# zhaozijie2022/LocoTouch

Measured on AMD Instinct MI355X. Metric: env-steps/sec (whole node), TransportTeacher 4096 envs/GPU, higher is better.
Workload: dtype f32

## Files before the change

locotouch_amd/_abi.py:

```python
from __future__ import annotations

import ctypes
import os
import re

_HERE = os.path.dirname(os.path.abspath(__file__))
REPO = os.path.dirname(_HERE)
LIB_PATH = os.environ.get("LOCOTOUCH_AMD_LIB", os.path.join(_HERE, "_lib", "liblocotouch_env.so"))

_SCALARS = {"int": ctypes.c_int, "int32_t": ctypes.c_int32, "int64_t": ctypes.c_int64, "uint8_t": ctypes.c_uint8,
            "uint32_t": ctypes.c_uint32, "uint64_t": ctypes.c_uint64, "size_t": ctypes.c_size_t, "float": ctypes.c_float,
            "double": ctypes.c_double}
_DECL = re.compile(r"(?:const\s+)?(\w+)\s*((?:\*\s*(?:const\b\s*)?)*)(\w*)\s*((?:\[[^\]]*\]\s*)*)")


def _ctype(decl, structs, opaque, consts, typed, param):
    m = _DECL.fullmatch(decl.strip())
    if not m:
        return None
    base, stars, name, dims = m.groups()
    depth = stars.count("*")
    try:
        dims = [sum(int(t) if t.strip().isdigit() else consts[t.strip()] for t in d.split("+")) for d in re.findall(r"\[([^\]]*)\]", dims)]
    except KeyError:
# ... 91 lines not shown
    ("MEMORY_GRU", "lt_memory_gru.h", False, ("lt_memory_gru_seq_backward_units",),
     ("lt_memory_gru_net", "lt_memory_gru_seq_net", "lt_memory_gru_seq_grad")),
    ("POLICY", "lt_policy.h", True, ("lt_policy_step_launches",), ("lt_policy_desc", "lt_policy_memory")),
    ("PPO_OPTS", "lt_ppo_opts.h", False, (), ()),
    ("MLP_DX", "lt_mlp_dx.h", True, (), ()),
    ("PPO_SYM", "lt_ppo_sym.h", False, (), ()),
    ("PPO_MIRROR", "lt_ppo_mirror.h", False, (), ()),
    ("MLP_ROWS", "lt_mlp_rows.h", True, (), ()),
    ("ENCODER", "lt_encoder.h", False, ("lt_encoder_forward_launches",), ("lt_encoder_desc", "lt_encoder_net")),
    ("RNN_ENCODER", "lt_rnn_encoder.h", False, ("lt_rnn_encoder_forward_launches",),
     ("lt_rnn_encoder_memory", "lt_rnn_encoder_net")),
    ("RNN_ENCODER_TRAIN", "lt_rnn_encoder_train.h", "lt_rnn_encoder.h", ("lt_rnn_encoder_backward_launches",),
     ("lt_rnn_encoder_grad",)),
    ("POLICY_ENCODER", "lt_policy_encoder.h", False, ("lt_policy_encoder_step_launches",),
     ("lt_policy_encoder_desc", "lt_policy_encoder_params")),
)


def _bind(table, include_dir):
    bound, seen, env_structs, structs_of = [], set(), None, {}
    for prefix, fname, uses_env_structs, queries, _ in table:
        path, queries = os.path.join(include_dir, fname), frozenset(queries)
        given = structs_of[uses_env_structs] if isinstance(uses_env_structs, str) else env_structs if uses_env_structs else None
        consts, structs, sigs = parse_header(open(path).read(), structs=given, bases={"lt_cfg": _CfgMethods})
        structs_of[fname] = structs
        if not prefix:
            env_structs = structs
        for name in sorted(queries - set(sigs)):
            raise ImportError(f"include/{fname}: the value query {name} named in _abi.HEADERS is not declared there")
        for name, (restype, _) in sigs.items():
# ... 117 lines not shown
```

locotouch_amd/csrc/lt_ppo.hip:

```cpp
#include <hip/hip_runtime.h>
#include <math.h>
#include <stdint.h>

#include "lt_env.h"
#include "lt_host_check.h"
#include "lt_internal.h"
#include "lt_ppo_device.h"

namespace {

template <bool LOG, bool NORM>
__global__ __launch_bounds__(256) void lt_ppo_loss_kernel(const float* __restrict__ mu, const float* __restrict__ stdp, const float* __restrict__ value,
                                                          const float* __restrict__ actions, const float* __restrict__ old_logp,
                                                          const float* __restrict__ adv, const float* __restrict__ returns,
                                                          const float* __restrict__ old_values, const float* __restrict__ old_mu,
                                                          const float* __restrict__ old_sigma, const long long* __restrict__ idx,
                                                          long long M, int A, float clip, float vcoef, int clipped_value,
                                                          const float* __restrict__ adv_stats, float* __restrict__ dmu, float* __restrict__ dvalue, float* __restrict__ acc) {
  const long long row = (long long)blockIdx.x * 256 + threadIdx.x;
  const bool ok = row < M;
  const long long src = (ok && idx) ? idx[row] : row;
  __shared__ float sigma_lds[MAX_A];
  if constexpr (LOG) {
    if ((int)threadIdx.x < A) sigma_lds[threadIdx.x] = lt_sigma_of_log(stdp[threadIdx.x]);
// ... 157 lines not shown
      else if (J.out1[j]) J.out1[j][ei - split] = o[i];
    }
  }
}

void launch_one_sum(const float* ws, int nblk, long long stride, int count, int split, float* out0, float* out1, hipStream_t stream) {
  SumJobs J = {};
  J.njobs = 1;
  J.ws[0] = ws; J.out0[0] = out0; J.out1[0] = out1; J.stride[0] = stride;
  J.nblk[0] = nblk; J.count[0] = count; J.split[0] = split;
  const int epb = 256 / sum_row_lanes(nblk) * 4;
  J.first[1] = (count + epb - 1) / epb;
  hipLaunchKernelGGL(lt_partial_sums_kernel, dim3((unsigned)J.first[1]), dim3(256), 0, stream, J);
}

constexpr int HW_ROWS = 96, HW_MAX_N = 16;

template <int NN>
__global__ __launch_bounds__(256) void lt_head_wgrad_kernel(const float* __restrict__ dy, const float* __restrict__ x, int x_split, long long M, int n, int k,
                                                            float* __restrict__ ws) {
  const int k4 = k >> 2, lanes = 256 / k4;
  const int c4 = threadIdx.x % k4, rl = threadIdx.x / k4;
  const long long r0 = (long long)blockIdx.x * HW_ROWS;
  float4 acc[NN];
  float accb[NN];
#pragma unroll
  for (int j = 0; j < NN; ++j) { acc[j] = {0.f, 0.f, 0.f, 0.f}; accb[j] = 0.f; }
  if (rl < lanes) {
    for (int r = rl; r < HW_ROWS; r += 4 * lanes) {
      float4 xv[4];
      float d[4][NN];
#pragma unroll
      for (int u = 0; u < 4; ++u) {
        const long long row = r0 + r + u * lanes;
        const bool ok = (r + u * lanes) < HW_ROWS && row < M;
        xv[u] = ok ? ((const float4*)(x + row * k))[c4] : float4{0.f, 0.f, 0.f, 0.f};
        if (x_split) {
          const unsigned w[4] = {__float_as_uint(xv[u].x), __float_as_uint(xv[u].y), __float_as_uint(xv[u].z), __float_as_uint(xv[u].w)};
          float f[4];
#pragma unroll
          for (int i = 0; i < 4; ++i)
            f[i] = (float)__builtin_bit_cast(_Float16, (unsigned short)(w[i] & 0xFFFFu)) + (float)__builtin_bit_cast(_Float16, (unsigned short)(w[i] >> 16)) * (1.f / 64.f);
          xv[u] = float4{f[0], f[1], f[2], f[3]};
        }
#pragma unroll
        for (int j = 0; j < NN; ++j) d[u][j] = (ok && j < n) ? dy[row * n + j] : 0.f;
      }
#pragma unroll
      for (int u = 0; u < 4; ++u)
#pragma unroll
        for (int j = 0; j < NN; ++j) {
          acc[j].x += d[u][j] * xv[u].x; acc[j].y += d[u][j] * xv[u].y; acc[j].z += d[u][j] * xv[u].z; acc[j].w += d[u][j] * xv[u].w;
          accb[j] += d[u][j];
        }
    }
  }
  extern __shared__ float4 red[];
  float* const redb = (float*)(red + (size_t)lanes * NN * k4);
  if (rl < lanes) {
#pragma unroll
    for (int j = 0; j < NN; ++j) red[((size_t)rl * NN + j) * k4 + c4] = acc[j];
    if (c4 == 0)
#pragma unroll
      for (int j = 0; j < NN; ++j) redb[rl * NN + j] = accb[j];
  }
  __syncthreads();
  float* const out = ws + (size_t)blockIdx.x * ((size_t)n * k + HW_MAX_N);
  for (int e = threadIdx.x; e < n * k4; e += 256) {
    const int j = e / k4, c = e - j * k4;
    float4 t = red[(size_t)j * k4 + c];
    for (int l = 1; l < lanes; ++l) {
      const float4 u = red[((size_t)l * NN + j) * k4 + c];
      t.x += u.x; t.y += u.y; t.z += u.z; t.w += u.w;
    }
    ((float4*)(out + (size_t)j * k))[c] = t;
  }
  if (threadIdx.x < n) {
    float t = redb[threadIdx.x];
    for (int l = 1; l < lanes; ++l) t += redb[l * NN + threadIdx.x];
    out[(size_t)n * k + threadIdx.x] = t;
  }
}

__global__ __launch_bounds__(256) void lt_gae_kernel(const float* __restrict__ rewards, const unsigned char* __restrict__ dones,
                                                     const float* __restrict__ values, const float* __restrict__ last_values, float gamma,
                                                     float lam, int T, long long N, float* __restrict__ returns, float* __restrict__ advantages) {
  const long long e = (long long)blockIdx.x * 256 + threadIdx.x;
  if (e >= N) return;
  float next_v = last_values[e], gae = 0.f;
  for (int t = T - 1; t >= 0; --t) {
    const long long o = (long long)t * N + e;
    const float v = values[o], alive = 1.f - (float)dones[o];
    const float delta = rewards[o] + alive * gamma * next_v - v;
    gae = delta + alive * gamma * lam * gae;
    const float ret = gae + v;
    returns[o] = ret;
// ... 122 lines not shown
}
static int elu_backward_bias(const float* da, const float* a, int64_t M, int N, float alpha, float* dz, float* db, float* ws, float* amax, void* stream) {
  if (!da || !a || !dz || !ws || M < 1 || N < 4 || (N & 3) || N > 1024)
    return einval("lt_elu_backward_bias: invalid argument (N a multiple of 4, 4 <= N <= 1024)");
  const int nblk = (int)((M + EB_ROWS - 1) / EB_ROWS);
  hipLaunchKernelGGL(lt_elu_bwd_bias_kernel, dim3((unsigned)nblk), dim3(256), 0, (hipStream_t)stream, da, a, (long long)M, N, alpha, dz, ws, amax);
  if (db) launch_one_sum(ws, nblk, (long long)N, N, N, db, nullptr, (hipStream_t)stream);
  return launch_status();
}

extern "C" int64_t lt_head_wgrad_ws_floats(int64_t M, int n, int k) { return ((M + HW_ROWS - 1) / HW_ROWS) * ((int64_t)n * k + HW_MAX_N); }

extern "C" int lt_head_wgrad(const float* dy, const float* x, int x_split, int64_t M, int n, int k, float* dw, float* db, float* ws, void* stream) {
  if (!dy || !x || !ws || M < 1 || n < 1 || n > HW_MAX_N || k < 4 || (k & 3) || k > 1024)
    return einval("lt_head_wgrad: invalid argument (1 <= n <= 16, k a multiple of 4, 4 <= k <= 1024)");
  const int nblk = (int)((M + HW_ROWS - 1) / HW_ROWS), k4 = k / 4, lanes = 256 / k4;
  const int nn = n <= 1 ? 1 : (n <= 4 ? 4 : (n <= 8 ? 8 : (n <= 12 ? 12 : 16)));
  const size_t lds = (size_t)lanes * nn * k4 * 16 + (size_t)lanes * nn * 4;
  if (const int e = lt_ensure_dynamic_lds((const void*)lt_head_wgrad_kernel<16>, 72 * 1024)) {
    lt_set_error(hipGetErrorString((hipError_t)e));
    return LT_EHIP;
  }
  if (lds > 72 * 1024) return einval("lt_head_wgrad: n * k too large for one block's LDS partials");
  const dim3 g((unsigned)nblk), b(256);
  hipStream_t st = (hipStream_t)stream;
  switch (nn) {
    case 1: hipLaunchKernelGGL(lt_head_wgrad_kernel<1>, g, b, lds, st, dy, x, x_split, (long long)M, n, k, ws); break;
    case 4: hipLaunchKernelGGL(lt_head_wgrad_kernel<4>, g, b, lds, st, dy, x, x_split, (long long)M, n, k, ws); break;
    case 8: hipLaunchKernelGGL(lt_head_wgrad_kernel<8>, g, b, lds, st, dy, x, x_split, (long long)M, n, k, ws); break;
    case 12: hipLaunchKernelGGL(lt_head_wgrad_kernel<12>, g, b, lds, st, dy, x, x_split, (long long)M, n, k, ws); break;
    default: hipLaunchKernelGGL(lt_head_wgrad_kernel<16>, g, b, lds, st, dy, x, x_split, (long long)M, n, k, ws); break;
  }
  if (dw) launch_one_sum(ws, nblk, (long long)n * k + HW_MAX_N, n * k + n, n * k, dw, db, st);
// ... 134 lines not shown
```

locotouch_amd/rl/flat_adam.py:

```python
from __future__ import annotations

import torch

from .. import _abi


class FlatAdam:
    ALIGN = 64

    def __init__(self, optimizer: torch.optim.Adam):
        if type(optimizer) is not torch.optim.Adam or len(optimizer.param_groups) != 1:
            raise TypeError("FlatAdam wraps a single-group torch.optim.Adam")
        g = optimizer.param_groups[0]
        if g.get("amsgrad") or g.get("maximize") or g.get("capturable") or g.get("differentiable"):
            raise TypeError("FlatAdam: amsgrad / maximize / capturable / differentiable are not supported")
        self.optimizer = optimizer
        self.params = [p for p in g["params"] if p.requires_grad]
        if not self.params or any(p.dtype != torch.float32 or not p.is_cuda for p in self.params):
            raise TypeError("FlatAdam needs f32 CUDA parameters")
        self.offsets, off = [], 0
        for p in self.params:
            self.offsets.append(off)
            off += -(-p.numel() // self.ALIGN) * self.ALIGN
        self.n = off
# ... 56 lines not shown
        return self.flat_g

    def grad_views(self) -> dict:
        if not self._bound():
            self._adopt()
        for p, v in zip(self.params, self._gviews):
            p.grad = v
        return {p: v for p, v in zip(self.params, self._gviews)}

    def offset_of(self, param) -> int:
        for p, off in zip(self.params, self.offsets):
            if p is param:
                return off
        raise KeyError("parameter not in the flat bucket")

    def step_dev(self, max_norm: float, lr_dev: torch.Tensor) -> None:
        if not self._bound():
            self._adopt()
        g = self.optimizer.param_groups[0]
        self.step_count += 1
        b1, b2 = g["betas"]
        _abi.call("lt_adam_clip_step_dev", self.flat_p, self.flat_g, self.flat_m, self.flat_v, self.n, float(max_norm or 0.0), lr_dev,
                  float(b1), float(b2), float(g["eps"]), float(g["weight_decay"]), self.step_count, self._ws, self.grad_norm,
                  _abi.stream(self.flat_p.device))
        self._step_t.fill_(float(self.step_count))

    def step(self, max_norm: float, gathered: bool = False) -> None:
        if not self._bound():
            self._adopt()
        if not gathered:
            self.gather_grads()
        g = self.optimizer.param_groups[0]
        self.step_count += 1
        b1, b2 = g["betas"]
        _abi.call("lt_adam_clip_step", self.flat_p, self.flat_g, self.flat_m, self.flat_v, self.n, float(max_norm or 0.0), float(g["lr"]),
                  float(b1), float(b2), float(g["eps"]), float(g["weight_decay"]), self.step_count, self._ws, self.grad_norm,
                  _abi.stream(self.flat_p.device))
        self._step_t.fill_(float(self.step_count))
```

locotouch_amd/rl/mlp.py:

```python
from __future__ import annotations

import ctypes
import os

import torch
import torch.nn as nn

from .. import _abi

USE_FUSED_BACKWARD = os.environ.get("LT_FUSED_BACKWARD", "1") != "0"
USE_DX_KERNEL = os.environ.get("LT_MLP_DX_KERNEL", "1") != "0"
_ACT_IDS = {nn.ELU: "LT_ACT_ELU", nn.ReLU: "LT_ACT_RELU", nn.Tanh: "LT_ACT_TANH", nn.Identity: "LT_ACT_NONE"}


def describe(seq: nn.Sequential):
    linears, acts = [], set()
    mods = list(seq)
    for i, m in enumerate(mods):
        if isinstance(m, nn.Linear):
            if m.bias is None or m.weight.dtype != torch.float32:
                return None
            linears.append(m)
        elif type(m) in _ACT_IDS:
            if type(m) is nn.ELU and (m.alpha != 1.0):
# ... 231 lines not shown
            torch.mm(dz.detach(), w.detach(), out=dx_out)


class PackedPair:

    def __init__(self, actor: nn.Sequential, critic: nn.Sequential):
        self.a, self.b = PackedMLP(actor), PackedMLP(critic)
        self.check_domain = False
        self.domain_max: torch.Tensor | None = None
        self.acts_split = False
        self._bpacked_fresh = False
        self._dx_fresh = False
        self.last_backward: str | None = None
        self._bwd_shapes_ok: bool | None = None
        self.sat: torch.Tensor | None = None
        for net in (self.a, self.b):
            dims = [net.desc.dims[i] for i in range(net.desc.num_layers + 1)]
            if any(d % 4 for d in dims[1:-1]) or net.desc.activation != _abi.CONSTS["LT_ACT_ELU"]:
                raise ValueError("PackedPair: ELU stacks with hidden widths that are multiples of 4")

    def arm_domain_check(self) -> None:
        self.check_domain = True

    def _record_domain(self, tensors) -> None:
        self.check_domain = False
        with torch.no_grad():
            m_ = torch.stack([t.abs().max().float() for t in tensors]).max()
            self.domain_max = m_ if self.domain_max is None else torch.maximum(self.domain_max, m_)

    def domain_violated(self) -> bool:
# ... 74 lines not shown
            x_split_rows, xsp = (self.split_rows(x0), self.split_rows(x1)), 1
        if xsp:
            xs = x_split_rows
        dys = [d if d.is_contiguous() else d.contiguous() for d in (dy0, dy1)]
        dev = x0.device
        if self.sat is None:
            self.sat = torch.zeros(1, device=dev, dtype=torch.float32)
        if ms[0] == ms[1]:
            nblks = (lib.lt_mlp_backward_blocks(ctypes.byref(nets[0].desc), ctypes.byref(nets[1].desc), ms[0]),) * 2
        else:
            if dx_out is not None:
                raise ValueError("PackedPair: input gradients (dx_out) are served for inputs of equal row counts only")
            blocks = (ctypes.c_int64(), ctypes.c_int64())
            _abi.call("lt_mlp_backward_blocks_rows", nets[0].desc, nets[1].desc, ms[0], ms[1], ctypes.byref(blocks[0]), ctypes.byref(blocks[1]))
            nblks = (blocks[0].value, blocks[1].value)
        dzs, amaxs, arrs = [], [], []
        per_net = (SumJobs(), SumJobs()) if after_first is not None else (sums, sums)
        for k, net in enumerate(nets):
            if not self._bpacked_fresh:
                net.pack_backward()
            L = len(net.linears)
            m, nblk = ms[k], nblks[k]
            n, kk = dys[k].shape[1], acts[k][L - 2].shape[1]
            ws = torch.empty(lib.lt_head_wgrad_ws_floats(m, n, kk), device=dev, dtype=torch.float32)
            _abi.call("lt_head_wgrad", dys[k], acts[k][L - 2], asp, m, n, kk, None, None, ws, stream)
            per_net[k].add(ws, lib.lt_head_wgrad_nblk(m), n * kk + 16, n * kk + n, n * kk, grad_of[net.linears[L - 1].weight], grad_of[net.linears[L - 1].bias])
            dz = [torch.empty_like(a) for a in acts[k]]
            am = torch.empty(L - 1, nblk, device=dev, dtype=torch.float32)
            dzs.append(dz)
            amaxs.append(am)
            arrs.append((_abi.ptr_array(acts[k]), _abi.ptr_array(dz), _abi.ptr_array([am[l] for l in range(L - 1)])))
        dzsp = int(dy_amax is not None)
        scales = torch.empty(2, device=dev, dtype=torch.float32)
        in_amax = dy_amax if dzsp else (None, None)
        dx_kernel = dx_out is not None and self._dx_kernel_ok()
        if dx_kernel and not self._dx_fresh:
            self.pack_training(with_backward=True, with_dx=True)
        chain = (nets[0].desc, nets[0].bpacked, dys[0], *arrs[0], nets[1].desc, nets[1].bpacked, dys[1], *arrs[1],
                 *(ms[:1] if ms[0] == ms[1] else ms), asp, in_amax[0], in_amax[1], dzsp, scales, self.sat)
        if ms[0] != ms[1]:
            _abi.call("lt_mlp_backward_pair_rows", *chain, stream)
        elif dx_kernel:
            _abi.call("lt_mlp_backward_pair_dx", *chain, dx_out[0], dx_out[1], stream)
        else:
            _abi.call("lt_mlp_backward_pair", *chain, stream)
            if dx_out is not None:
# ... 56 lines not shown
```

locotouch_amd/rl/ppo.py:

```python
from __future__ import annotations

import torch
import torch.nn as nn

from .. import _abi
from .dist import Dist
from .modules import ActorCritic
from .storage import RolloutStorage


class PPO:
    def __init__(self, actor_critic: ActorCritic, num_learning_epochs=1, num_mini_batches=1, clip_param=0.2, gamma=0.998,
                 lam=0.95, value_loss_coef=1.0, entropy_coef=0.0, learning_rate=1e-3, max_grad_norm=1.0,
                 use_clipped_value_loss=True, schedule="fixed", desired_kl=0.01, device="cpu",
                 normalize_advantage_per_mini_batch=False, dist: Dist | None = None, rnd_cfg: dict | None = None,
                 symmetry_cfg: dict | None = None, **unused):
        if rnd_cfg is not None:
            raise NotImplementedError("rnd_cfg: random network distillation is not built (DESIGN.md §7: it needs an `rnd_state` observation "
                                      "group no env here produces); pass rnd_cfg=None")
        self.symmetry = self._resolve_symmetry(symmetry_cfg, actor_critic)
        self._sym_tables = None
        self.device = device
        self.dist = dist or Dist()
        self.actor_critic = actor_critic.to(device)
        on_gpu = torch.device(device).type == "cuda"
        self.fused_loss = on_gpu and bool(unused.get("fused_loss", True))
        self.packed_forward = on_gpu and bool(unused.get("packed_forward", True))
        self.direct_update = on_gpu and bool(unused.get("direct_update", True))
        self.fused_recurrent_update = bool(unused.get("fused_recurrent_update", False))
        self.fused_gru_memories = bool(unused.get("fused_gru_memories", False))
        self.direct_recurrent_update = bool(unused.get("direct_recurrent_update", False))
        self.fused_encoder_policy = bool(unused.get("fused_encoder_policy", False))
        self._encoders = None
        self.direct_rnn_encoder_update = bool(unused.get("direct_rnn_encoder_update", False))
        self._rnn_encoders = None
        if type(actor_critic).__name__ == "ActorCriticRNNEncoder":
            for key in ("fused_encoder_policy", "direct_recurrent_update", "fused_recurrent_update"):
                if getattr(self, key):
                    raise ValueError(f"{key}: the policy is an ActorCriticRNNEncoder: its update is the eager one (the key serves "
                                     f"{'ActorCriticEncoder' if key == 'fused_encoder_policy' else 'ActorCriticRecurrent'})")
        if self.fused_encoder_policy:
            if self.fused_recurrent_update or self.direct_recurrent_update or self.fused_gru_memories:
                raise ValueError("fused_encoder_policy: the recurrent keys (fused_recurrent_update, direct_recurrent_update, fused_gru_memories) "
# ... 198 lines not shown
            if self._adaptive:
                self._apply_kl(self.dist.all_reduce_mean_end(kl_handle), reduced=True)
            self._optim_step()
            stats = stats + torch.stack((value_loss, surrogate_loss, ent.detach()))
        n = self.num_learning_epochs * self.num_mini_batches
        sv, ss, se = (stats / n).tolist()
        if pair is not None and pair.domain_violated():
            self._warn_mlp_domain()
        st.clear()
        return sv, ss, se, None, None

    def _direct_update(self, pair, split_buckets: bool = True):
        ac, fa, sym = self.actor_critic, self._flat_adam, self.symmetry
        perm, m = self.storage.mini_batch_permutation(self.num_mini_batches)
        c = self._direct_begin("direct_update", pair, perm, m, symmetric=sym is not None)
        obs, cobs, dev, grad_of = c.obs, c.cobs, c.dev, c.grad_of
        critic_at = fa.offset_of(next(iter(ac.critic.parameters())))
        two_buckets = split_buckets and 0 < critic_at < self._flat_grad.numel()
        sym_args = None
        mirror_only = sym is not None and not sym["use_data_augmentation"]
        if sym is None:
            rows = crows = m
            perm_o, perm_co = obs[perm], cobs[perm]
            if perm_o.dtype != torch.float32:
                perm_o, perm_co = perm_o.float(), perm_co.float()
        elif mirror_only:
            rows, crows = 2 * m, m
            tab_o, _, tab_a = self._symmetry_tables(dev, obs.shape[1], None, c.a_dim)
            perm_o, perm_co = self._symmetry_gather(obs, perm, m, tab_o), cobs[perm]
            if perm_co.dtype != torch.float32:
# ... 14 lines not shown
            (mu, value), acts = pair.forward_raw(o, co)
            dmu, dvalue, acc = self._direct_loss_and_rule(c, mu, value, idx, m, i, sym_args)
            if brows != rows:
                o, dmu, acts = o[:brows], dmu[:brows], ([a[:brows] for a in acts[0]], acts[1])
            if self.dist.world_size > 1 and two_buckets:
                handles = []
                pair.backward_raw(o, co, acts, dmu, dvalue, grad_of, xs, after_first=lambda: handles.append(self.dist.all_reduce_mean_begin(self._flat_grad[:critic_at])),
                                  dy_amax=(acc[20:21], acc[21:22]))
                handles.append(self.dist.all_reduce_mean_begin(self._flat_grad[critic_at:] if handles else self._flat_grad))
                for h in handles:
                    self.dist.all_reduce_mean_end(h)
            else:
                pair.backward_raw(o, co, acts, dmu, dvalue, grad_of, xs, dy_amax=(acc[20:21], acc[21:22]))
                if self.dist.world_size > 1:
                    self.dist.all_reduce_mean_(self._flat_grad)
            fa.step_dev(self.max_grad_norm, c.lr_dev)
        return self._direct_end(c, with_dx=False)

    def _direct_begin(self, key: str, pair, index, m: int, symmetric: bool = False):
        from types import SimpleNamespace

        from .fused_loss import adv_stats, std_param

        obs, cobs, small = self._flat_storage()
        small = [t.view(-1) if t.shape[-1] == 1 else t for t in small]
        a_dim = small[0].shape[1]
        if a_dim > 16:
            raise ValueError(f"{key}: the action width is {a_dim}: the loss kernel serves at most 16")
        dev = obs.device
        state = torch.zeros(5 if symmetric else 4, device=dev)
        state[0] = self.learning_rate
        std_p, std_is_log = std_param(self.actor_critic)
        pair.arm_domain_check()
        mb_stats = adv_stats(small[2], index, m, self.num_mini_batches) if self.normalize_advantage_per_mini_batch else None
        return SimpleNamespace(pair=pair, obs=obs, cobs=cobs, small=small, a_dim=a_dim, dev=dev, state=state, lr_dev=state[:1], stats=state[1:4],
                               grad_of=self._flat_adam.grad_views(), std_p=std_p, std_is_log=std_is_log, std_c=std_p.detach(),
                               stream=_abi.stream(dev), mb_stats=mb_stats)

    def _direct_loss_and_rule(self, c, mu, value, idx, m: int, i: int, sym_args=None):
        dev = c.dev
        dmu = torch.empty_like(mu)
        dvalue = torch.empty(value.shape[0], 1, device=dev, dtype=torch.float32)
        acc = torch.empty(24, device=dev, dtype=torch.float32)
        out = torch.empty(24, device=dev, dtype=torch.float32)
        rows = (mu, c.std_c, value, *c.small, idx, m, c.a_dim, float(self.clip_param), float(self.value_loss_coef), float(self.entropy_coef),
                int(bool(self.use_clipped_value_loss)))
        opts = (int(c.std_is_log), None if c.mb_stats is None else c.mb_stats[i])
        if sym_args is not None:
            _abi.call(sym_args[0], *rows, *opts, *sym_args[1:], dmu, dvalue, acc, out, c.state[4:5], c.stream)
        elif c.std_is_log or c.mb_stats is not None:
            _abi.call("lt_ppo_loss_opts", *rows, *opts, dmu, dvalue, acc, out, c.stream)
        else:
            _abi.call("lt_ppo_loss", *rows, dmu, dvalue, acc, out, c.stream)
        kl = None
        if self._adaptive:
            kl = out[4:5]
            if self.dist.world_size > 1:
                kl = self.dist.all_reduce_mean_(kl.clone())
        _abi.call("lt_ppo_lr_rule", kl, float(self.desired_kl or 0.0), 1e-5, 1e-2, 1.5, c.lr_dev, c.stats, out, c.grad_of[c.std_p], c.a_dim, c.stream)
        return dmu, dvalue, acc

    def _direct_end(self, c, with_dx: bool):
        pair, state = c.pair, c.state
        sat, dom = pair.saturated(), pair.domain_max
        pair.domain_max = None
        zero = state.new_zeros(1)
        read = torch.cat((state, zero if sat is None else sat, zero if dom is None else dom.view(1))).tolist()
        (lr, sv, ss, se), (nsat, dmax) = read[:4], read[-2:]
        if nsat > 0:
            import warnings

            sat.zero_()
            entry = "lt_mlp_backward_pair_dx" if with_dx and pair._dx_kernel_ok() else "lt_mlp_backward_pair"
            warnings.warn(f"{entry}: {int(nsat)} workgroup-layers of the gradient chain reached the f16 image's bound "
                          "(a gradient grew by more than 500x through the layers): those rows were saturated; set LT_FUSED_BACKWARD=0 "
                          "to run the chain as f32 library GEMMs")
        self.learning_rate = lr
        for group in self.optimizer.param_groups:
# ... 545 lines not shown
```

Baseline: 68.62 million.

## Fuse PPO loss, partial sums and LR rule into one step; pair head wgrad launches

Adds a new loss-step entry point. It computes the PPO loss rows, staging per-row tensors through LDS tiles, and writes per-block partials. A tail kernel then reduces those partials and applies the adaptive LR rule and std gradient, replacing the separate loss, sum and lr_rule launches. The two networks' head weight-gradient kernels are merged into one paired launch, and the Adam step-count publish moves to once per update instead of every mini-batch. The aim is to cut kernel launches and host overhead per mini-batch, at the cost of new code paths that only apply to the non-symmetric, non-log-std, no-per-minibatch-norm case.

```diff
diff --git a/include/lt_ppo_step.h b/include/lt_ppo_step.h
--- /dev/null
+++ b/include/lt_ppo_step.h
@@ -0,0 +1,26 @@
+#ifndef LT_PPO_STEP_H
+#define LT_PPO_STEP_H
+
+#include <stddef.h>
+#include <stdint.h>
+
+#ifdef __cplusplus
+extern "C" {
+#endif
+
+int lt_ppo_loss_step_ws_floats(int64_t M);
+
+int lt_ppo_loss_step(const float* mu, const float* std, const float* value, const float* actions, const float* old_logp, const float* adv,
+                     const float* returns, const float* old_values, const float* old_mu, const float* old_sigma, const int64_t* idx, int64_t M,
+                     int A, float clip, float value_loss_coef, float entropy_coef, int use_clipped_value_loss, int std_is_log,
+                     const float* adv_stats, float desired_kl, float lr_min, float lr_max, float factor, float* lr, float* stats,
+                     float* dstd_out, float* dmu, float* dvalue, float* partials, float* acc, float* out, void* stream);
+
+int lt_head_wgrad_pair(const float* dy0, const float* x0, int64_t M0, int n0, int k0, float* ws0, const float* dy1, const float* x1, int64_t M1,
+                       int n1, int k1, float* ws1, int x_split, void* stream);
+
+#ifdef __cplusplus
+}
+#endif
+
+#endif
diff --git a/locotouch_amd/_abi.py b/locotouch_amd/_abi.py
--- a/locotouch_amd/_abi.py
+++ b/locotouch_amd/_abi.py
@@ -129,6 +129,7 @@
      ("lt_rnn_encoder_grad",)),
     ("POLICY_ENCODER", "lt_policy_encoder.h", False, ("lt_policy_encoder_step_launches",),
      ("lt_policy_encoder_desc", "lt_policy_encoder_params")),
+    ("PPO_STEP", "lt_ppo_step.h", False, ("lt_ppo_loss_step_ws_floats",), ()),
 )
 
 
diff --git a/locotouch_amd/csrc/lt_head_wgrad_device.h b/locotouch_amd/csrc/lt_head_wgrad_device.h
--- /dev/null
+++ b/locotouch_amd/csrc/lt_head_wgrad_device.h
@@ -0,0 +1,80 @@
+#pragma once
+
+#include <hip/hip_runtime.h>
+
+namespace {
+
+constexpr int HW_ROWS = 96, HW_MAX_N = 16;
+
+template <int NN>
+__device__ __forceinline__ void lt_head_wgrad_block(const float* __restrict__ dy, const float* __restrict__ x, int x_split, long long M, int n, int k,
+                                                    float* __restrict__ ws, long long blk, float4* red) {
+  const int k4 = k >> 2, lanes = 256 / k4;
+  const int c4 = threadIdx.x % k4, rl = threadIdx.x / k4;
+  const long long r0 = blk * HW_ROWS;
+  float4 acc[NN];
+  float accb[NN];
+#pragma unroll
+  for (int j = 0; j < NN; ++j) { acc[j] = {0.f, 0.f, 0.f, 0.f}; accb[j] = 0.f; }
+  if (rl < lanes) {
+    for (int r = rl; r < HW_ROWS; r += 4 * lanes) {
+      float4 xv[4];
+      float d[4][NN];
+#pragma unroll
+      for (int u = 0; u < 4; ++u) {
+        const long long row = r0 + r + u * lanes;
+        const bool ok = (r + u * lanes) < HW_ROWS && row < M;
+        xv[u] = ok ? ((const float4*)(x + row * k))[c4] : float4{0.f, 0.f, 0.f, 0.f};
+        if (x_split) {
+          const unsigned w[4] = {__float_as_uint(xv[u].x), __float_as_uint(xv[u].y), __float_as_uint(xv[u].z), __float_as_uint(xv[u].w)};
+          float f[4];
+#pragma unroll
+          for (int i = 0; i < 4; ++i)
+            f[i] = (float)__builtin_bit_cast(_Float16, (unsigned short)(w[i] & 0xFFFFu)) + (float)__builtin_bit_cast(_Float16, (unsigned short)(w[i] >> 16)) * (1.f / 64.f);
+          xv[u] = float4{f[0], f[1], f[2], f[3]};
+        }
+#pragma unroll
+        for (int j = 0; j < NN; ++j) d[u][j] = (ok && j < n) ? dy[row * n + j] : 0.f;
+      }
+#pragma unroll
+      for (int u = 0; u < 4; ++u)
+#pragma unroll
+        for (int j = 0; j < NN; ++j) {
+          acc[j].x += d[u][j] * xv[u].x; acc[j].y += d[u][j] * xv[u].y; acc[j].z += d[u][j] * xv[u].z; acc[j].w += d[u][j] * xv[u].w;
+          accb[j] += d[u][j];
+        }
+    }
+  }
+  float* const redb = (float*)(red + (size_t)lanes * NN * k4);
+  if (rl < lanes) {
+#pragma unroll
+    for (int j = 0; j < NN; ++j) red[((size_t)rl * NN + j) * k4 + c4] = acc[j];
+    if (c4 == 0)
+#pragma unroll
+      for (int j = 0; j < NN; ++j) redb[rl * NN + j] = accb[j];
+  }
+  __syncthreads();
+  float* const out = ws + (size_t)blk * ((size_t)n * k + HW_MAX_N);
+  for (int e = threadIdx.x; e < n * k4; e += 256) {
+    const int j = e / k4, c = e - j * k4;
+    float4 t = red[(size_t)j * k4 + c];
+    for (int l = 1; l < lanes; ++l) {
+      const float4 u = red[((size_t)l * NN + j) * k4 + c];
+      t.x += u.x; t.y += u.y; t.z += u.z; t.w += u.w;
+    }
+    ((float4*)(out + (size_t)j * k))[c] = t;
+  }
+  if (threadIdx.x < n) {
+    float t = redb[threadIdx.x];
+    for (int l = 1; l < lanes; ++l) t += redb[l * NN + threadIdx.x];
+    out[(size_t)n * k + threadIdx.x] = t;
+  }
+}
+
+__host__ __device__ inline int lt_head_wgrad_nn(int n) { return n <= 1 ? 1 : (n <= 4 ? 4 : (n <= 8 ? 8 : (n <= 12 ? 12 : 16))); }
+inline size_t lt_head_wgrad_lds(int n, int k) {
+  const int k4 = k / 4, lanes = 256 / k4, nn = lt_head_wgrad_nn(n);
+  return (size_t)lanes * nn * k4 * 16 + (size_t)lanes * nn * 4;
+}
+
+}
diff --git a/locotouch_amd/csrc/lt_ppo.hip b/locotouch_amd/csrc/lt_ppo.hip
--- a/locotouch_amd/csrc/lt_ppo.hip
+++ b/locotouch_amd/csrc/lt_ppo.hip
@@ -3,6 +3,7 @@
 #include <stdint.h>
 
 #include "lt_env.h"
+#include "lt_head_wgrad_device.h"
 #include "lt_host_check.h"
 #include "lt_internal.h"
 #include "lt_ppo_device.h"
@@ -195,72 +196,11 @@
   hipLaunchKernelGGL(lt_partial_sums_kernel, dim3((unsigned)J.first[1]), dim3(256), 0, stream, J);
 }
 
-constexpr int HW_ROWS = 96, HW_MAX_N = 16;
-
 template <int NN>
 __global__ __launch_bounds__(256) void lt_head_wgrad_kernel(const float* __restrict__ dy, const float* __restrict__ x, int x_split, long long M, int n, int k,
                                                             float* __restrict__ ws) {
-  const int k4 = k >> 2, lanes = 256 / k4;
-  const int c4 = threadIdx.x % k4, rl = threadIdx.x / k4;
-  const long long r0 = (long long)blockIdx.x * HW_ROWS;
-  float4 acc[NN];
-  float accb[NN];
-#pragma unroll
-  for (int j = 0; j < NN; ++j) { acc[j] = {0.f, 0.f, 0.f, 0.f}; accb[j] = 0.f; }
-  if (rl < lanes) {
-    for (int r = rl; r < HW_ROWS; r += 4 * lanes) {
-      float4 xv[4];
-      float d[4][NN];
-#pragma unroll
-      for (int u = 0; u < 4; ++u) {
-        const long long row = r0 + r + u * lanes;
-        const bool ok = (r + u * lanes) < HW_ROWS && row < M;
-        xv[u] = ok ? ((const float4*)(x + row * k))[c4] : float4{0.f, 0.f, 0.f, 0.f};
-        if (x_split) {
-          const unsigned w[4] = {__float_as_uint(xv[u].x), __float_as_uint(xv[u].y), __float_as_uint(xv[u].z), __float_as_uint(xv[u].w)};
-          float f[4];
-#pragma unroll
-          for (int i = 0; i < 4; ++i)
-            f[i] = (float)__builtin_bit_cast(_Float16, (unsigned short)(w[i] & 0xFFFFu)) + (float)__builtin_bit_cast(_Float16, (unsigned short)(w[i] >> 16)) * (1.f / 64.f);
-          xv[u] = float4{f[0], f[1], f[2], f[3]};
-        }
-#pragma unroll
-        for (int j = 0; j < NN; ++j) d[u][j] = (ok && j < n) ? dy[row * n + j] : 0.f;
-      }
-#pragma unroll
-      for (int u = 0; u < 4; ++u)
-#pragma unroll
-        for (int j = 0; j < NN; ++j) {
-          acc[j].x += d[u][j] * xv[u].x; acc[j].y += d[u][j] * xv[u].y; acc[j].z += d[u][j] * xv[u].z; acc[j].w += d[u][j] * xv[u].w;
-          accb[j] += d[u][j];
-        }
-    }
-  }
   extern __shared__ float4 red[];
-  float* const redb = (float*)(red + (size_t)lanes * NN * k4);
-  if (rl < lanes) {
-#pragma unroll
-    for (int j = 0; j < NN; ++j) red[((size_t)rl * NN + j) * k4 + c4] = acc[j];
-    if (c4 == 0)
-#pragma unroll
-      for (int j = 0; j < NN; ++j) redb[rl * NN + j] = accb[j];
-  }
-  __syncthreads();
-  float* const out = ws + (size_t)blockIdx.x * ((size_t)n * k + HW_MAX_N);
-  for (int e = threadIdx.x; e < n * k4; e += 256) {
-    const int j = e / k4, c = e - j * k4;
-    float4 t = red[(size_t)j * k4 + c];
-    for (int l = 1; l < lanes; ++l) {
-      const float4 u = red[((size_t)l * NN + j) * k4 + c];
-      t.x += u.x; t.y += u.y; t.z += u.z; t.w += u.w;
-    }
-    ((float4*)(out + (size_t)j * k))[c] = t;
-  }
-  if (threadIdx.x < n) {
-    float t = redb[threadIdx.x];
-    for (int l = 1; l < lanes; ++l) t += redb[l * NN + threadIdx.x];
-    out[(size_t)n * k + threadIdx.x] = t;
-  }
+  lt_head_wgrad_block<NN>(dy, x, x_split, M, n, k, ws, (long long)blockIdx.x, red);
 }
 
 __global__ __launch_bounds__(256) void lt_gae_kernel(const float* __restrict__ rewards, const unsigned char* __restrict__ dones,
@@ -413,9 +353,8 @@
 extern "C" int lt_head_wgrad(const float* dy, const float* x, int x_split, int64_t M, int n, int k, float* dw, float* db, float* ws, void* stream) {
   if (!dy || !x || !ws || M < 1 || n < 1 || n > HW_MAX_N || k < 4 || (k & 3) || k > 1024)
     return einval("lt_head_wgrad: invalid argument (1 <= n <= 16, k a multiple of 4, 4 <= k <= 1024)");
-  const int nblk = (int)((M + HW_ROWS - 1) / HW_ROWS), k4 = k / 4, lanes = 256 / k4;
-  const int nn = n <= 1 ? 1 : (n <= 4 ? 4 : (n <= 8 ? 8 : (n <= 12 ? 12 : 16)));
-  const size_t lds = (size_t)lanes * nn * k4 * 16 + (size_t)lanes * nn * 4;
+  const int nblk = (int)((M + HW_ROWS - 1) / HW_ROWS), nn = lt_head_wgrad_nn(n);
+  const size_t lds = lt_head_wgrad_lds(n, k);
   if (const int e = lt_ensure_dynamic_lds((const void*)lt_head_wgrad_kernel<16>, 72 * 1024)) {
     lt_set_error(hipGetErrorString((hipError_t)e));
     return LT_EHIP;
diff --git a/locotouch_amd/csrc/lt_ppo_step.hip b/locotouch_amd/csrc/lt_ppo_step.hip
--- /dev/null
+++ b/locotouch_amd/csrc/lt_ppo_step.hip
@@ -0,0 +1,311 @@
+#include <hip/hip_runtime.h>
+#include <math.h>
+#include <stdint.h>
+
+#include "lt_env.h"
+#include "lt_head_wgrad_device.h"
+#include "lt_host_check.h"
+#include "lt_internal.h"
+#include "lt_ppo_device.h"
+#include "lt_ppo_step.h"
+
+namespace {
+
+constexpr int LS_ROWS = 256;
+constexpr int LS_SLOTS = 24;
+constexpr int LS_WAVES = LS_ROWS / 64;
+constexpr int LS_TAIL_CHUNK = 128;
+
+__host__ __device__ inline int ls_stride(int A, int vec) { return vec ? (((A >> 2) & 1) ? A : A + 4) : (A | 1); }
+
+template <bool TO_LDS, typename G>
+__device__ __forceinline__ void ls_move_rows(float* __restrict__ tile, G g, int nrows, int A, int S, int vec) {
+  if (vec) {
+    const int a4 = A >> 2, nq = nrows * a4;
+    for (int q = threadIdx.x; q < nq; q += LS_ROWS) {
+      const int r = q / a4, p = q - r * a4;
+      float4* const l = (float4*)(tile + r * S + 4 * p);
+      if constexpr (TO_LDS) *l = *(const float4*)(g(r) + 4 * p);
+      else *(float4*)(g(r) + 4 * p) = *l;
+    }
+  } else {
+    const int ne = nrows * A;
+    for (int e = threadIdx.x; e < ne; e += LS_ROWS) {
+      const int r = e / A, a = e - r * A;
+      if constexpr (TO_LDS) tile[r * S + a] = g(r)[a];
+      else g(r)[a] = tile[r * S + a];
+    }
+  }
+}
+
+__device__ __forceinline__ void ls_own_row(const float* __restrict__ tile, int A, int S, int vec, float (&o)[MAX_A]) {
+  const float* const p = tile + (int)threadIdx.x * S;
+  if (vec) {
+#pragma unroll
+    for (int c = 0; c < MAX_A / 4; ++c) {
+      if (4 * c < A) {
+        const float4 v = *(const float4*)(p + 4 * c);
+        o[4 * c] = v.x; o[4 * c + 1] = v.y; o[4 * c + 2] = v.z; o[4 * c + 3] = v.w;
+      }
+    }
+  } else {
+#pragma unroll
+    for (int a = 0; a < MAX_A; ++a)
+      if (a < A) o[a] = p[a];
+  }
+}
+
+__device__ __forceinline__ float ls_inv_sigma(float sg) {
+#pragma clang fp reciprocal(off)
+  return 1.f / sg;
+}
+
+template <bool LOG, bool NORM>
+__global__ __launch_bounds__(LS_ROWS) void lt_ppo_loss_rows_kernel(const float* __restrict__ mu, const float* __restrict__ stdp, const float* __restrict__ value,
+                                                                   const float* __restrict__ actions, const float* __restrict__ old_logp,
+                                                                   const float* __restrict__ adv, const float* __restrict__ returns,
+                                                                   const float* __restrict__ old_values, const float* __restrict__ old_mu,
+                                                                   const float* __restrict__ old_sigma, const long long* __restrict__ idx,
+                                                                   long long M, int A, float clip, float vcoef, int clipped_value,
+                                                                   const float* __restrict__ adv_stats, int vec, float* __restrict__ dmu,
+                                                                   float* __restrict__ dvalue, float* __restrict__ partials) {
+  extern __shared__ float4 tiles4[];
+  __shared__ long long s_src[LS_ROWS];
+  __shared__ float sigma_lds[MAX_A];
+  __shared__ float red[LS_WAVES][4 + MAX_A];
+  __shared__ float redm[LS_WAVES][2];
+  const int S = ls_stride(A, vec);
+  float* const t_mu = (float*)tiles4;
+  float* const t_act = t_mu + LS_ROWS * S;
+  float* const t_omu = t_act + LS_ROWS * S;
+  float* const t_osg = t_omu + LS_ROWS * S;
+  const long long r0 = (long long)blockIdx.x * LS_ROWS, row = r0 + threadIdx.x;
+  const int nrows = (int)(M - r0 < LS_ROWS ? M - r0 : LS_ROWS);
+  const bool ok = (int)threadIdx.x < nrows;
+  const long long src = (ok && idx) ? idx[row] : row;
+  s_src[threadIdx.x] = src;
+  if constexpr (LOG) {
+    if ((int)threadIdx.x < A) sigma_lds[threadIdx.x] = lt_sigma_of_log(stdp[threadIdx.x]);
+  }
+  float v = 0.f, R = 0.f, olp = 0.f, advr = 0.f, ov_own = 0.f;
+  if (ok) { v = value[row]; R = returns[src]; olp = old_logp[src]; advr = adv[src]; ov_own = old_values[src]; }
+  const float* const mu_blk = mu + r0 * A;
+  ls_move_rows<true>(t_mu, [&](int r) { return mu_blk + (long long)r * A; }, nrows, A, S, vec);
+  __syncthreads();
+  ls_move_rows<true>(t_act, [&](int r) { return actions + s_src[r] * A; }, nrows, A, S, vec);
+  ls_move_rows<true>(t_omu, [&](int r) { return old_mu + s_src[r] * A; }, nrows, A, S, vec);
+  ls_move_rows<true>(t_osg, [&](int r) { return old_sigma + s_src[r] * A; }, nrows, A, S, vec);
+  __syncthreads();
+  float part[4 + MAX_A];
+  float amax_mu = 0.f, amax_v = 0.f;
+#pragma unroll
+  for (int i = 0; i < 4 + MAX_A; ++i) part[i] = 0.f;
+  if (ok) {
+    const float inv_m = 1.f / (float)M;
+    float logp = 0.f, kl = 0.f;
+    float z[MAX_A], isg[MAX_A], rm[MAX_A], rx[MAX_A], rom[MAX_A], ros[MAX_A];
+    ls_own_row(t_mu, A, S, vec, rm);
+    ls_own_row(t_act, A, S, vec, rx);
+    ls_own_row(t_omu, A, S, vec, rom);
+    ls_own_row(t_osg, A, S, vec, ros);
+#pragma unroll
+    for (int a = 0; a < MAX_A; ++a) {
+      if (a < A) {
+        const float sg = LOG ? sigma_lds[a] : stdp[a], m = rm[a], x = rx[a];
+        const float om = rom[a], os = ros[a];
+        isg[a] = ls_inv_sigma(sg);
+        z[a] = (x - m) * isg[a];
+        logp += lt_ppo_logp_term<LOG>(z[a], sg, stdp[a]);
+        kl += lt_ppo_kl_term(sg, os, om, m);
+      }
+    }
+    if constexpr (NORM) advr = (advr - adv_stats[0]) * adv_stats[1];
+    const float ratio = __expf(logp - olp);
+    LT_PPO_SURROGATE(advr, ratio, clip, s1, s2, dsurr_dratio)
+    const float dlogp = dsurr_dratio * ratio * inv_m;
+    float* const my_dmu = t_mu + (int)threadIdx.x * S;
+#pragma unroll
+    for (int a = 0; a < MAX_A; ++a) {
+      if (a < A) {
+        my_dmu[a] = dlogp * z[a] * isg[a];
+        amax_mu = fmaxf(amax_mu, fabsf(dlogp * z[a] * isg[a]));
+        if constexpr (LOG) part[4 + a] = dlogp * (z[a] * z[a] - 1.f);
+        else part[4 + a] = dlogp * (z[a] * z[a] - 1.f) * isg[a];
+      }
+    }
+    float vl, dv;
+    LT_PPO_VALUE_LOSS(v, R, &ov_own, 0, clip, clipped_value, vl, dv)
+    dvalue[row] = vcoef * dv * inv_m;
+    amax_v = fabsf(vcoef * dv * inv_m);
+    part[0] = fmaxf(s1, s2);
+    part[1] = vl;
+    part[2] = kl;
+  }
+  const int lane = threadIdx.x & 63, wave = threadIdx.x >> 6;
+#pragma unroll
+  for (int i = 0; i < 4 + MAX_A; ++i) {
+    float s = part[i];
+#pragma unroll
+    for (int off = 32; off > 0; off >>= 1) s += __shfl_xor(s, off, 64);
+    if (lane == 0) red[wave][i] = s;
+  }
+#pragma unroll
+  for (int off = 32; off > 0; off >>= 1) {
+    amax_mu = fmaxf(amax_mu, __shfl_xor(amax_mu, off, 64));
+    amax_v = fmaxf(amax_v, __shfl_xor(amax_v, off, 64));
+  }
+  if (lane == 0) { redm[wave][0] = amax_mu; redm[wave][1] = amax_v; }
+  __syncthreads();
+  float* const dmu_blk = dmu + r0 * A;
+  ls_move_rows<false>(t_mu, [&](int r) { return dmu_blk + (long long)r * A; }, nrows, A, S, vec);
+  if (threadIdx.x < LS_SLOTS) {
+    const int i = threadIdx.x;
+    float s = 0.f;
+    if (i < 4 + A && i != 3) {
+      s = red[0][i];
+#pragma unroll
+      for (int w = 1; w < LS_WAVES; ++w) s += red[w][i];
+    } else if (i == 20 || i == 21) {
+#pragma unroll
+      for (int w = 0; w < LS_WAVES; ++w) s = fmaxf(s, redm[w][i - 20]);
+    }
+    partials[(long long)blockIdx.x * LS_SLOTS + i] = s;
+  }
+}
+
+__global__ __launch_bounds__(256) void lt_ppo_loss_tail_kernel(const float* __restrict__ partials, int nblk, const float* __restrict__ stdp, int A, float inv_m,
+                                                               float vcoef, float ecoef, int std_is_log, float desired, float lr_min, float lr_max,
+                                                               float factor, float* __restrict__ lr, float* __restrict__ stats,
+                                                               float* __restrict__ dstd_out, float* __restrict__ acc, float* __restrict__ out) {
+  __shared__ float s_part[LS_TAIL_CHUNK * LS_SLOTS];
+  __shared__ float s_acc[LS_SLOTS], s_out[LS_SLOTS];
+  const int t = threadIdx.x;
+  const bool is_max = t == 20 || t == 21;
+  float s = 0.f;
+  for (int b0 = 0; b0 < nblk; b0 += LS_TAIL_CHUNK) {
+    const int nb = nblk - b0 < LS_TAIL_CHUNK ? nblk - b0 : LS_TAIL_CHUNK;
+    for (int e = t; e < nb * LS_SLOTS; e += 256) s_part[e] = partials[(long long)b0 * LS_SLOTS + e];
+    __syncthreads();
+    if (t < LS_SLOTS) {
+      if (is_max) for (int b = 0; b < nb; ++b) s = fmaxf(s, s_part[b * LS_SLOTS + t]);
+      else for (int b = 0; b < nb; ++b) s += s_part[b * LS_SLOTS + t];
+    }
+    __syncthreads();
+  }
+  if (t < LS_SLOTS) { s_acc[t] = s; acc[t] = s; s_out[t] = 0.f; }
+  __syncthreads();
+  if (t < 64) lt_ppo_finalize(s_acc, stdp, A, inv_m, vcoef, ecoef, std_is_log, s_out);
+  __syncthreads();
+  if (out && (t < 5 || (t >= 8 && t < 8 + A))) out[t] = s_out[t];
+  if (dstd_out && t < A) dstd_out[t] = s_out[8 + t];
+  if (t != 0) return;
+  if (lr && desired > 0.f) {
+#pragma clang fp reciprocal(off)
+    const float kl = s_out[4];
+    float v = *lr;
+    if (kl > desired * 2.f) v = fmaxf(lr_min, v / factor);
+    else if (kl < desired * 0.5f && kl > 0.f) v = fminf(lr_max, v * factor);
+    *lr = v;
+  }
+  if (stats) { stats[0] += s_out[2]; stats[1] += s_out[1]; stats[2] += s_out[3]; }
+}
+
+struct HeadPair {
+  const float *dy0, *x0, *dy1, *x1;
+  float *ws0, *ws1;
+  long long M0, M1;
+  int n0, k0, n1, k1, nblk0, x_split;
+};
+
+__global__ __launch_bounds__(256) void lt_head_wgrad_pair_kernel(const HeadPair P) {
+  extern __shared__ float4 red[];
+  const bool second = (int)blockIdx.x >= P.nblk0;
+  const float* const dy = second ? P.dy1 : P.dy0;
+  const float* const x = second ? P.x1 : P.x0;
+  float* const ws = second ? P.ws1 : P.ws0;
+  const long long M = second ? P.M1 : P.M0, blk = (long long)blockIdx.x - (second ? P.nblk0 : 0);
+  const int n = second ? P.n1 : P.n0, k = second ? P.k1 : P.k0;
+  switch (lt_head_wgrad_nn(n)) {
+    case 1: lt_head_wgrad_block<1>(dy, x, P.x_split, M, n, k, ws, blk, red); break;
+    case 4: lt_head_wgrad_block<4>(dy, x, P.x_split, M, n, k, ws, blk, red); break;
+    case 8: lt_head_wgrad_block<8>(dy, x, P.x_split, M, n, k, ws, blk, red); break;
+    case 12: lt_head_wgrad_block<12>(dy, x, P.x_split, M, n, k, ws, blk, red); break;
+    default: lt_head_wgrad_block<16>(dy, x, P.x_split, M, n, k, ws, blk, red); break;
+  }
+}
+
+}
+
+constexpr int64_t LS_MAX_ROWS = (int64_t)(0x7fffffff / LS_SLOTS) * LS_ROWS;
+
+extern "C" int lt_ppo_loss_step_ws_floats(int64_t M) { return M < 1 || M > LS_MAX_ROWS ? -1 : (int)((M + LS_ROWS - 1) / LS_ROWS * LS_SLOTS); }
+
+extern "C" int lt_ppo_loss_step(const float* mu, const float* stdp, const float* value, const float* actions, const float* old_logp, const float* adv,
+                                const float* returns, const float* old_values, const float* old_mu, const float* old_sigma, const int64_t* idx,
+                                int64_t M, int A, float clip, float value_loss_coef, float entropy_coef, int use_clipped_value_loss, int std_is_log,
+                                const float* adv_stats, float desired_kl, float lr_min, float lr_max, float factor, float* lr, float* stats,
+                                float* dstd_out, float* dmu, float* dvalue, float* partials, float* acc, float* out, void* stream) {
+  const char* fn = "lt_ppo_loss_step";
+  const ptr_check ptrs[] = {{"mu", mu, 4}, {"std", stdp, 4}, {"value", value, 4}, {"actions", actions, 4}, {"old_logp", old_logp, 4}, {"adv", adv, 4},
+                            {"returns", returns, 4}, {"old_values", old_values, 4}, {"old_mu", old_mu, 4}, {"old_sigma", old_sigma, 4},
+                            {"dmu", dmu, 4}, {"dvalue", dvalue, 4}, {"partials", partials, 4}, {"acc", acc, 4}};
+  if (const int rc = check_ptrs(fn, "", ptrs)) return rc;
+  if ((uintptr_t)idx % 8 != 0) return refuse(fn, "", "idx", "NULL or 8-byte aligned");
+  const ptr_check optional[] = {{"adv_stats", adv_stats, 4}, {"lr", lr, 4}, {"stats", stats, 4}, {"dstd_out", dstd_out, 4}, {"out", out, 4}};
+  for (const auto& e : optional)
+    if ((uintptr_t)e.p % 4 != 0) return refuse(fn, "", e.name, "NULL or 4-byte aligned");
+  if (M < 1 || M > LS_MAX_ROWS) return refuse(fn, "", "M", "in [1, 22906492160]");
+  if (A < 1 || A > MAX_A) return refuse(fn, "", "A", "in [1, 16]");
+  if (lr && !(factor > 1.f)) return refuse(fn, "", "factor", "> 1 where lr is given");
+  const int64_t nblk = (M + LS_ROWS - 1) / LS_ROWS;
+  int vec = A % 4 == 0;
+  for (const void* p : {(const void*)mu, (const void*)actions, (const void*)old_mu, (const void*)old_sigma, (const void*)dmu})
+    vec = vec && (uintptr_t)p % 16 == 0;
+  const size_t lds = (size_t)4 * LS_ROWS * ls_stride(A, vec) * sizeof(float);
+  const void* kernel = std_is_log ? (adv_stats ? (const void*)lt_ppo_loss_rows_kernel<true, true> : (const void*)lt_ppo_loss_rows_kernel<true, false>)
+                                  : (adv_stats ? (const void*)lt_ppo_loss_rows_kernel<false, true> : (const void*)lt_ppo_loss_rows_kernel<false, false>);
+  if (const int e = lt_ensure_dynamic_lds(kernel, (int)((size_t)4 * LS_ROWS * (MAX_A + 4) * sizeof(float)))) {
+    lt_set_error(hipGetErrorString((hipError_t)e));
+    return LT_EHIP;
+  }
+  const dim3 grid((unsigned)nblk);
+  hipStream_t st = (hipStream_t)stream;
+#define LT_PPO_ROWS_LAUNCH(LOG, NORM)                                                                                                            \
+  hipLaunchKernelGGL((lt_ppo_loss_rows_kernel<LOG, NORM>), grid, dim3(LS_ROWS), lds, st, mu, stdp, value, actions, old_logp, adv, returns, old_values, \
+                     old_mu, old_sigma, (const long long*)idx, (long long)M, A, clip, value_loss_coef, use_clipped_value_loss, adv_stats, vec, dmu,  \
+                     dvalue, partials)
+  if (std_is_log && adv_stats) LT_PPO_ROWS_LAUNCH(true, true);
+  else if (std_is_log) LT_PPO_ROWS_LAUNCH(true, false);
+  else if (adv_stats) LT_PPO_ROWS_LAUNCH(false, true);
+  else LT_PPO_ROWS_LAUNCH(false, false);
+#undef LT_PPO_ROWS_LAUNCH
+  hipLaunchKernelGGL(lt_ppo_loss_tail_kernel, dim3(1), dim3(256), 0, st, partials, (int)nblk, stdp, A, 1.f / (float)M, value_loss_coef, entropy_coef,
+                     std_is_log ? 1 : 0, desired_kl, lr_min, lr_max, factor, lr, stats, dstd_out, acc, out);
+  return launch_status(fn);
+}
+
+extern "C" int lt_head_wgrad_pair(const float* dy0, const float* x0, int64_t M0, int n0, int k0, float* ws0, const float* dy1, const float* x1, int64_t M1,
+                                  int n1, int k1, float* ws1, int x_split, void* stream) {
+  const char* fn = "lt_head_wgrad_pair";
+  const ptr_check ptrs[] = {{"dy0", dy0, 4}, {"x0", x0, 16}, {"ws0", ws0, 16}, {"dy1", dy1, 4}, {"x1", x1, 16}, {"ws1", ws1, 16}};
+  if (const int rc = check_ptrs(fn, "", ptrs)) return rc;
+  const struct { const char* who; int64_t M; int n, k; } nets[2] = {{"network 0: ", M0, n0, k0}, {"network 1: ", M1, n1, k1}};
+  size_t lds = 0;
+  for (const auto& t : nets) {
+    if (t.M < 1) return refuse(fn, t.who, "M", ">= 1");
+    if (t.n < 1 || t.n > HW_MAX_N) return refuse(fn, t.who, "n", "in [1, 16]");
+    if (t.k < 4 || (t.k & 3) || t.k > 1024) return refuse(fn, t.who, "k", "a multiple of 4 in [4, 1024]");
+    if ((t.M + HW_ROWS - 1) / HW_ROWS > 0x3fffffff) return refuse(fn, t.who, "M", "at most 2^30 - 1 blocks of 96 rows");
+    const size_t l = lt_head_wgrad_lds(t.n, t.k);
+    if (l > 72 * 1024) return refuse(fn, t.who, "n * k", "small enough for one block's LDS partials (as lt_head_wgrad)");
+    lds = l > lds ? l : lds;
+  }
+  if (const int e = lt_ensure_dynamic_lds((const void*)lt_head_wgrad_pair_kernel, 72 * 1024)) {
+    lt_set_error(hipGetErrorString((hipError_t)e));
+    return LT_EHIP;
+  }
+  HeadPair P = {dy0, x0, dy1, x1, ws0, ws1, (long long)M0, (long long)M1, n0, k0, n1, k1, (int)((M0 + HW_ROWS - 1) / HW_ROWS), x_split ? 1 : 0};
+  const unsigned nblk = (unsigned)P.nblk0 + (unsigned)((M1 + HW_ROWS - 1) / HW_ROWS);
+  hipLaunchKernelGGL(lt_head_wgrad_pair_kernel, dim3(nblk), dim3(256), lds, (hipStream_t)stream, P);
+  return launch_status(fn);
+}
diff --git a/locotouch_amd/rl/flat_adam.py b/locotouch_amd/rl/flat_adam.py
--- a/locotouch_amd/rl/flat_adam.py
+++ b/locotouch_amd/rl/flat_adam.py
@@ -94,7 +94,10 @@
                 return off
         raise KeyError("parameter not in the flat bucket")
 
-    def step_dev(self, max_norm: float, lr_dev: torch.Tensor) -> None:
+    def publish_step(self) -> None:
+        self._step_t.fill_(float(self.step_count))
+
+    def step_dev(self, max_norm: float, lr_dev: torch.Tensor, publish: bool = True) -> None:
         if not self._bound():
             self._adopt()
         g = self.optimizer.param_groups[0]
@@ -103,7 +106,8 @@
         _abi.call("lt_adam_clip_step_dev", self.flat_p, self.flat_g, self.flat_m, self.flat_v, self.n, float(max_norm or 0.0), lr_dev,
                   float(b1), float(b2), float(g["eps"]), float(g["weight_decay"]), self.step_count, self._ws, self.grad_norm,
                   _abi.stream(self.flat_p.device))
-        self._step_t.fill_(float(self.step_count))
+        if publish:
+            self.publish_step()
 
     def step(self, max_norm: float, gathered: bool = False) -> None:
         if not self._bound():
diff --git a/locotouch_amd/rl/mlp.py b/locotouch_amd/rl/mlp.py
--- a/locotouch_amd/rl/mlp.py
+++ b/locotouch_amd/rl/mlp.py
@@ -269,6 +269,7 @@
         self.last_backward: str | None = None
         self._bwd_shapes_ok: bool | None = None
         self.sat: torch.Tensor | None = None
+        self.head_pair = True
         for net in (self.a, self.b):
             dims = [net.desc.dims[i] for i in range(net.desc.num_layers + 1)]
             if any(d % 4 for d in dims[1:-1]) or net.desc.activation != _abi.CONSTS["LT_ACT_ELU"]:
@@ -373,7 +374,7 @@
             blocks = (ctypes.c_int64(), ctypes.c_int64())
             _abi.call("lt_mlp_backward_blocks_rows", nets[0].desc, nets[1].desc, ms[0], ms[1], ctypes.byref(blocks[0]), ctypes.byref(blocks[1]))
             nblks = (blocks[0].value, blocks[1].value)
-        dzs, amaxs, arrs = [], [], []
+        dzs, amaxs, arrs, heads = [], [], [], []
         per_net = (SumJobs(), SumJobs()) if after_first is not None else (sums, sums)
         for k, net in enumerate(nets):
             if not self._bpacked_fresh:
@@ -382,13 +383,17 @@
             m, nblk = ms[k], nblks[k]
             n, kk = dys[k].shape[1], acts[k][L - 2].shape[1]
             ws = torch.empty(lib.lt_head_wgrad_ws_floats(m, n, kk), device=dev, dtype=torch.float32)
-            _abi.call("lt_head_wgrad", dys[k], acts[k][L - 2], asp, m, n, kk, None, None, ws, stream)
+            heads += [dys[k], acts[k][L - 2], m, n, kk, ws]
+            if not self.head_pair:
+                _abi.call("lt_head_wgrad", dys[k], acts[k][L - 2], asp, m, n, kk, None, None, ws, stream)
             per_net[k].add(ws, lib.lt_head_wgrad_nblk(m), n * kk + 16, n * kk + n, n * kk, grad_of[net.linears[L - 1].weight], grad_of[net.linears[L - 1].bias])
             dz = [torch.empty_like(a) for a in acts[k]]
             am = torch.empty(L - 1, nblk, device=dev, dtype=torch.float32)
             dzs.append(dz)
             amaxs.append(am)
             arrs.append((_abi.ptr_array(acts[k]), _abi.ptr_array(dz), _abi.ptr_array([am[l] for l in range(L - 1)])))
+        if self.head_pair:
+            _abi.call("lt_head_wgrad_pair", *heads, asp, stream)
         dzsp = int(dy_amax is not None)
         scales = torch.empty(2, device=dev, dtype=torch.float32)
         in_amax = dy_amax if dzsp else (None, None)
diff --git a/locotouch_amd/rl/ppo.py b/locotouch_amd/rl/ppo.py
--- a/locotouch_amd/rl/ppo.py
+++ b/locotouch_amd/rl/ppo.py
@@ -27,6 +27,7 @@
         self.fused_loss = on_gpu and bool(unused.get("fused_loss", True))
         self.packed_forward = on_gpu and bool(unused.get("packed_forward", True))
         self.direct_update = on_gpu and bool(unused.get("direct_update", True))
+        self.fused_loss_step = bool(unused.get("fused_loss_step", True))
         self.fused_recurrent_update = bool(unused.get("fused_recurrent_update", False))
         self.fused_gru_memories = bool(unused.get("fused_gru_memories", False))
         self.direct_recurrent_update = bool(unused.get("direct_recurrent_update", False))
@@ -255,6 +256,8 @@
         ac, fa, sym = self.actor_critic, self._flat_adam, self.symmetry
         perm, m = self.storage.mini_batch_permutation(self.num_mini_batches)
         c = self._direct_begin("direct_update", pair, perm, m, symmetric=sym is not None)
+        c.loss_step = self.fused_loss_step and sym is None and not c.std_is_log and c.mb_stats is None
+        pair.head_pair = self.fused_loss_step
         obs, cobs, dev, grad_of = c.obs, c.cobs, c.dev, c.grad_of
         critic_at = fa.offset_of(next(iter(ac.critic.parameters())))
         two_buckets = split_buckets and 0 < critic_at < self._flat_grad.numel()
@@ -299,7 +302,7 @@
                 pair.backward_raw(o, co, acts, dmu, dvalue, grad_of, xs, dy_amax=(acc[20:21], acc[21:22]))
                 if self.dist.world_size > 1:
                     self.dist.all_reduce_mean_(self._flat_grad)
-            fa.step_dev(self.max_grad_norm, c.lr_dev)
+            fa.step_dev(self.max_grad_norm, c.lr_dev, publish=False)
         return self._direct_end(c, with_dx=False)
 
     def _direct_begin(self, key: str, pair, index, m: int, symmetric: bool = False):
@@ -320,17 +323,30 @@
         mb_stats = adv_stats(small[2], index, m, self.num_mini_batches) if self.normalize_advantage_per_mini_batch else None
         return SimpleNamespace(pair=pair, obs=obs, cobs=cobs, small=small, a_dim=a_dim, dev=dev, state=state, lr_dev=state[:1], stats=state[1:4],
                                grad_of=self._flat_adam.grad_views(), std_p=std_p, std_is_log=std_is_log, std_c=std_p.detach(),
-                               stream=_abi.stream(dev), mb_stats=mb_stats)
+                               stream=_abi.stream(dev), mb_stats=mb_stats, loss_step=False, step_bufs=None)
 
     def _direct_loss_and_rule(self, c, mu, value, idx, m: int, i: int, sym_args=None):
         dev = c.dev
+        rows = (mu, c.std_c, value, *c.small, idx, m, c.a_dim, float(self.clip_param), float(self.value_loss_coef), float(self.entropy_coef),
+                int(bool(self.use_clipped_value_loss)))
+        opts = (int(c.std_is_log), None if c.mb_stats is None else c.mb_stats[i])
+        if c.loss_step:
+            if c.step_bufs is None or c.step_bufs[0].shape != mu.shape:
+                c.step_bufs = (torch.empty_like(mu), torch.empty(value.shape[0], 1, device=dev, dtype=torch.float32),
+                               torch.empty(_abi.load().lt_ppo_loss_step_ws_floats(m), device=dev, dtype=torch.float32),
+                               torch.empty(24, device=dev, dtype=torch.float32), torch.empty(24, device=dev, dtype=torch.float32))
+            dmu, dvalue, partials, acc, out = c.step_bufs
+            one_rank = self.dist.world_size == 1
+            rule = (float(self.desired_kl or 0.0) if self._adaptive else 0.0, 1e-5, 1e-2, 1.5, c.lr_dev if one_rank else None)
+            _abi.call("lt_ppo_loss_step", *rows, *opts, *rule, c.stats, c.grad_of[c.std_p], dmu, dvalue, partials, acc, out, c.stream)
+            if self._adaptive and not one_rank:
+                kl = self.dist.all_reduce_mean_(out[4:5].clone())
+                _abi.call("lt_ppo_lr_rule", kl, float(self.desired_kl or 0.0), 1e-5, 1e-2, 1.5, c.lr_dev, None, None, None, 0, c.stream)
+            return dmu, dvalue, acc
         dmu = torch.empty_like(mu)
         dvalue = torch.empty(value.shape[0], 1, device=dev, dtype=torch.float32)
         acc = torch.empty(24, device=dev, dtype=torch.float32)
         out = torch.empty(24, device=dev, dtype=torch.float32)
-        rows = (mu, c.std_c, value, *c.small, idx, m, c.a_dim, float(self.clip_param), float(self.value_loss_coef), float(self.entropy_coef),
-                int(bool(self.use_clipped_value_loss)))
-        opts = (int(c.std_is_log), None if c.mb_stats is None else c.mb_stats[i])
         if sym_args is not None:
             _abi.call(sym_args[0], *rows, *opts, *sym_args[1:], dmu, dvalue, acc, out, c.state[4:5], c.stream)
         elif c.std_is_log or c.mb_stats is not None:
@@ -347,6 +363,7 @@
 
     def _direct_end(self, c, with_dx: bool):
         pair, state = c.pair, c.state
+        self._flat_adam.publish_step()
         sat, dom = pair.saturated(), pair.domain_max
         pair.domain_max = None
         zero = state.new_zeros(1)
```

Result: no change. 68.34 million (-0.4%).
